# sz3/libcimbar

Hardware: AMD Instinct MI355X
Metric: decoded cimbar frames/s (1024x1024 mode-B) (higher is better)
Workload: dtype u8; 1 GPU; BASELINE configs[1]: 1024 clean mode-B frames per GPU per step, device-resident, bit-exact; distinct_input_batches=4, exchange_ranks=1, parallelism=frame-sharded x1; 3 steps in flight (pipelined entry point)

## Files before the change

### libcimbar_amd/csrc/host.hip.inc

```
struct CombineStream {
	DevBuf<uint8_t> symbols, colors, chunks; DevBuf<uint32_t> plane, flood, masks; DevBuf<int8_t> drift;
	DevBuf<uint32_t> weights;
	DevBuf<int> words;
	DevBuf<int> gsizes;
	Event ev_last;
	bool used = false;
	int min_agree = 0, max_group = 0;
	int vote = 0;
	CarryStore store() const { return CarryStore{symbols, colors, plane, drift, flood, chunks, masks, words, weights}; }
};

struct StitchStream {
	DevBuf<uint8_t> symbols, colors;
	DevBuf<uint32_t> usable;
	Event ev_last;
	bool used = false;
	bool carried = false;
	int cur = 0;
	StitchCarry carry() const { return StitchCarry{symbols, colors, usable, cur}; }
};

struct OnceStream {
	DevBuf<uint8_t> sig, row;
	DevBuf<uint32_t> words;
// ... 48 lines not shown
	DevBuf<uint8_t> d_rp_rchunks; DevBuf<uint32_t> d_rp_rmasks;
	int wave_adapt = 1;
	bool wave_ran = false;
	int wave_skip_left = 0;
	bool no_split_once = false;
	std::string err;
	Tables tb{};
	DevBuf<ushort2> tb_cell_xy; DevBuf<uint16_t> tb_stream_cell, tb_cell_grid, tb_ccm_grid; DevBuf<int16_t> tb_grid_cell, tb_cand;
	DevBuf<uint8_t> tb_stitch_line;
	DevBuf<uint16_t> tb_stitch_width;
	uint64_t tile_hashes[16] = {};
	int last_n = 0;
	int scan_n = 0;
	unsigned scan_w = 0, scan_h = 0;
	DevBuf<uint8_t> d_rgb;
	static constexpr int MAXP = 4;
	struct ScratchSet {
		int cap = 0;
		DevBuf<uint32_t> d_plane, d_cellmean;
		DevBuf<uint8_t> d_symbols, d_colors;
		DevBuf<int8_t> d_drift;
		DevBuf<uint32_t> d_flood;
		DevBuf<uint8_t> d_rs_ok;
		DevBuf<FrameState> d_states;
		DevBuf<float> d_ccm_frames, d_ccm_used;
		DevBuf<uint32_t> d_cmargin;
		int cm_cap = 0;
	} sets[MAXP];
	int pipe_depth = 3;
#ifdef CIMBAR_PROBES
	int dbg_skip = 0;
#else
	static constexpr int dbg_skip = 0;
#endif
	int pipe_set = 0;
	ScratchSet& cur() { return sets[pipe_set]; }
	bool pipe_used[MAXP] = {};
	Stream pstream_own[MAXP];
	hipStream_t pstream[MAXP] = {};
	Event ev_pk1[MAXP], ev_pdone[MAXP];
	Event ev_pgather[MAXP];
	bool pipe_gathered[MAXP] = {};
	struct FrameSlot {
		DevBuf<uint8_t> d_rgb;
		DevBuf<uint8_t> d_out;
		PinnedBuf<uint8_t> h_out;
		PinnedBuf<uint8_t> h_in;
		Event done;
		uint8_t* user_chunks = nullptr; uint32_t* user_mask = nullptr;
		long long ticket = -1;
	} fslot[MAXP];
	long long frame_tickets = 0;
	int k1_tall = -1;
	int k1_lds_pad = 0;
	size_t warp_scratch = (size_t)4 << 30;
	int warp_twopass = 1;
	DevBuf<int4> d_ex_box;
	DevBuf<uint8_t> d_ex_rgb;
	int frame_stage = 0;
	int frame_zerocopy = 1;
	int frame_copystream = 0;
	Stream fcopy;
	Event ev_fcopy[MAXP];
	struct FrameResult { long long ticket = -1; int rc = 0; } fresult[16];
	DevBuf<float> d_carry;
	DevBuf<uint8_t> d_template;
	DevBuf<uint8_t> d_gen_log;
	DevBuf<uint8_t> d_payload;
	DevBuf<uint8_t> d_chunks;
	DevBuf<uint32_t> d_masks;
	DevBuf<uint8_t> d_ex_in;
	const uint8_t* pad_src = nullptr; int pad_w = 0, pad_h = 0, pad_off = 0;
	DevBuf<uint8_t> d_ex_out;
	DevBuf<uint32_t> d_ex_hist; DevBuf<int> d_ex_thr; DevBuf<double> d_ex_minv;
	DevBuf<uint8_t> d_ex_gray;
	DevBuf<uint8_t> d_ex_frames;
	DevBuf<uint32_t> d_scan_hits; DevBuf<int> d_scan_nhits; DevBuf<ScanResult> d_scan_res;
	DevBuf<ScanAnchor> d_scan_serial;
	DevBuf<int> d_scan_offs, d_scan_ovf; DevBuf<ScanConf> d_scan_conf; DevBuf<ScanStage> d_scan_stage;
	PinnedBuf<double> h_ex_minv;
	Event ev_ex_minv;
	DevBuf<uint8_t> d_ud_img;
	DevBuf<int> d_ud_ok; DevBuf<double> d_ud_k1; DevBuf<int> d_ud_status;
	DevBuf<double> d_ud_xt; PinnedBuf<double> h_ud_xt;
	Event ev_ud_xt;
	size_t ud_scratch = (size_t)256 << 20;
	FloodScratch flood{};
	DevBuf<uint32_t> flood_heap, flood_next; DevBuf<uint8_t> flood_prio;
	int flood_cap = 0;
	DevBuf<uint32_t> d_fw_queue;
	int flood_verify = 0;
	DevBuf<uint8_t> d_vsym; DevBuf<int8_t> d_vdrift; DevBuf<uint32_t> d_vflag; int vcap = 0;
	DevBuf<unsigned long long> d_vtotals;
	int flood_dense_grid = 2048;
	int flood_dense = -1;
	int flood_wave = 1;
	int rf_threshold = -1, rf_fallback = 0;
	int rf_grid = FR_GRID;
	bool rf_valid = false;
	DevBuf<unsigned long long> d_rf_stats;
	bool timing = false;
	static constexpr int NSTAGE = 8;
	Event ev[NSTAGE + 1];
	float stage_ms[NSTAGE] = {};

	~cimbar_hip_ctx()
// ... 262 lines not shown
	ctx->vcap = 0;
	HIPCHK(ctx->d_vsym.reserve((size_t)n * NCELLS));
	HIPCHK(ctx->d_vdrift.reserve((size_t)n * NCELLS * 2));
	HIPCHK(ctx->d_vflag.reserve((size_t)n * 2));
	HIPCHK(hipMemset(ctx->d_vflag, 0xFF, sizeof(uint32_t) * (size_t)n * 2));
	if (!ctx->d_vtotals) { HIPCHK(ctx->d_vtotals.reserve(2)); HIPCHK(hipMemset(ctx->d_vtotals, 0, 2 * sizeof(unsigned long long))); }
	ctx->vcap = n;
	return 0;
}

int stage_input(cimbar_hip_ctx* ctx, hipStream_t st, DevBuf<uint8_t>& buf, const uint8_t* src, size_t bytes, int mem, const uint8_t** d)
{
	*d = src;
	if (mem == CIMBAR_HIP_MEM_HOST) {
		HIPCHK(buf.reserve(bytes));
		HIPCHK(hipMemcpyAsync(buf, src, bytes, hipMemcpyHostToDevice, st));
		*d = buf;
	}
	return 0;
}

int stage_output(cimbar_hip_ctx* ctx, DevBuf<uint8_t>& buf, uint8_t* dst, size_t bytes, int mem, uint8_t** d)
{
	*d = dst;
	if (mem == CIMBAR_HIP_MEM_HOST) {
		HIPCHK(buf.reserve(bytes));
		*d = buf;
	}
	return 0;
}

int drain_pipeline_into(cimbar_hip_ctx* ctx, hipStream_t st)
{
	for (int k = 0; k < cimbar_hip_ctx::MAXP; ++k)
		if (ctx->pipe_used[k]) HIPCHK(hipStreamWaitEvent(st, ctx->ev_pdone[k], 0));
	return 0;
}

void rotate_scratch_sets(cimbar_hip_ctx* ctx) { ctx->pipe_set = (ctx->pipe_set + 1) % ctx->pipe_depth; }

int ensure_flood_areas(cimbar_hip_ctx* ctx, int count)
{
	if (count <= ctx->flood_cap) return 0;
	HIPCHK(hipDeviceSynchronize());
	ctx->flood_cap = 0;
	HIPCHK(ctx->flood_heap.reserve((size_t)count * HEAP_CAP));
	HIPCHK(ctx->flood_prio.reserve((size_t)count * PRIO_STRIDE));
	if (!ctx->flood_next) { HIPCHK(ctx->flood_next.reserve((size_t)2 * FLOOD_COUNTERS)); HIPCHK(hipMemset(ctx->flood_next, 0, sizeof(uint32_t) * 2 * FLOOD_COUNTERS)); }
	ctx->flood = FloodScratch{ctx->flood_heap, ctx->flood_next, ctx->flood_prio};
	ctx->flood_cap = count;
	return 0;
}

constexpr int K1_TALL_MIN = 256;
constexpr int ERASURE_MAX_DEFAULT = RS_PARITY - 8;
inline int erasure_max(const cimbar_hip_ctx* ctx) { return ctx->er_max < 0 ? ERASURE_MAX_DEFAULT : ctx->er_max; }
inline int colour_erasure_max(const cimbar_hip_ctx* ctx) { return ctx->ec_max < 0 ? ERASURE_MAX_DEFAULT : ctx->ec_max; }

int enqueue(cimbar_hip_ctx* ctx, hipStream_t st, const uint8_t* d_rgb, int n, int pre, int cc, uint8_t* d_chunks, uint32_t* d_masks, int plain = 0,
            bool pipe = false, const int* d_sel = nullptr, int sel_stride = 0, bool symbols_only = false)
{
	cimbar_hip_ctx::ScratchSet& cur = ctx->cur();
	ctx->grp_valid = false;
	ctx->stitch_n = 0;
	ctx->gcv_valid = false;
	ctx->gcv_stream_n = -1;
	const bool colour_retry = !LEGACY && !plain && !symbols_only && ctx->ec_margin > 0;
	if (colour_retry) { if (int r = ensure_margin_capacity(ctx, cur)) return r; }
	ctx->cm_valid = colour_retry;
	const bool tm = ctx->timing && !pipe;
	int evi = 0;
	auto mark = [&]() -> hipError_t { return tm ? hipEventRecord(ctx->ev[evi++], st) : hipSuccess; };
	const dim3 cell_grid((NCELLS + 255) / 256, n);
	const int f0 = 0;

	uint32_t flagged[3] = {0, 0, 0};
	if (ctx->h_flagged) for (int k = 0; k < 3; ++k) flagged[k] = ((volatile uint32_t*)ctx->h_flagged)[k];
	const bool mostly_flood = flagged[1] != 0 && 4u * flagged[0] > flagged[1];
	const bool split = !tm && !pipe && ctx->tail_split && !ctx->no_split_once && !mostly_flood && n >= 64 * ctx->tail_parts;
	{
		const int areas_ = pipe ? FLOOD_GRID / ctx->pipe_depth : (split ? FLOOD_GRID / 2 : FLOOD_GRID);
		const int off_ = pipe ? (ctx->pipe_depth - 1) * areas_ : (split ? FLOOD_GRID / 2 : 0);
		int top = off_ + (n < areas_ ? n : areas_);
		if (ctx->flood_dense > 0 || (ctx->flood_dense < 0 && n > areas_)) top = FLOOD_DENSE_PER * off_ + (n < FLOOD_DENSE_PER * areas_ ? n : FLOOD_DENSE_PER * areas_);
		if (int r = ensure_flood_areas(ctx, top)) return r;
		if (ctx->flood_verify) if (int r = ensure_verify_capacity(ctx, n)) return r;
	}
	HIPCHK(mark());
	{
		dim3 g(K1_BLOCKS, n), gt(K1_TALL_BLOCKS, n);
		const bool pre_tall = ctx->k1_tall > 0 || (ctx->k1_tall < 0 && n >= K1_TALL_MIN);
		if (ctx->pad_src && n == 1) {
			uint8_t* frame = const_cast<uint8_t*>(d_rgb);
			const dim3 gp((IMG_W + 63) / 64, (IMG_H + 3) / 4);
			if (pre) hipLaunchKernelGGL((k_threshold_padded<3, true>), gp, dim3(256), 0, st, ctx->pad_src, ctx->pad_w, ctx->pad_h, ctx->pad_off, cur.d_plane, frame, cur.d_flood);
			else hipLaunchKernelGGL((k_threshold_padded<2, false>), gp, dim3(256), 0, st, ctx->pad_src, ctx->pad_w, ctx->pad_h, ctx->pad_off, cur.d_plane, frame, cur.d_flood);
			hipLaunchKernelGGL(k_cellmean_padded, dim3((GRID_CELLS + 255) / 256), dim3(256), 0, st, frame, cur.d_cellmean);
		} else if (d_sel) {
			if (pre_tall) hipLaunchKernelGGL((k_threshold<3, true, K1_TALLROWS>), gt, dim3(256), 0, st, d_rgb, cur.d_plane, cur.d_cellmean, cur.d_flood, f0, d_sel, sel_stride);
			else hipLaunchKernelGGL((k_threshold<3, true>), g, dim3(256), 0, st, d_rgb, cur.d_plane, cur.d_cellmean, cur.d_flood, f0, d_sel, sel_stride);
			hipLaunchKernelGGL((k_threshold<2, false>), g, dim3(256), 0, st, d_rgb, cur.d_plane, cur.d_cellmean, cur.d_flood, f0, d_sel, sel_stride);
		} else if (pre) {
			if (pre_tall) hipLaunchKernelGGL((k_threshold<3, true, K1_TALLROWS>), gt, dim3(256), 0, st, d_rgb, cur.d_plane, cur.d_cellmean, cur.d_flood, f0, (const int*)nullptr, 0);
			else hipLaunchKernelGGL((k_threshold<3, true>), g, dim3(256), 0, st, d_rgb, cur.d_plane, cur.d_cellmean, cur.d_flood, f0, (const int*)nullptr, 0);
		} else if (ctx->k1_tall > 0 || (ctx->k1_tall < 0 && pipe && n >= K1_TALL_MIN))
			hipLaunchKernelGGL((k_threshold<2, false, K1_TALLROWS>), dim3(K1_TALL_BLOCKS, n), dim3(256), (size_t)ctx->k1_lds_pad, st, d_rgb, cur.d_plane, cur.d_cellmean, cur.d_flood, f0, (const int*)nullptr, 0);
		else hipLaunchKernelGGL((k_threshold<2, false>), g, dim3(256), (size_t)ctx->k1_lds_pad, st, d_rgb, cur.d_plane, cur.d_cellmean, cur.d_flood, f0, (const int*)nullptr, 0);
	}
	HIPCHK(mark());
	const bool counted = !pipe && !tm && ctx->h_flagged && ctx->tail_split && n >= 64 * ctx->tail_parts;
	bool run_wave = ctx->flood_wave != 0;
	if (run_wave && counted && ctx->wave_adapt && !ctx->flood_verify) {
		if (ctx->wave_skip_left > 0) { --ctx->wave_skip_left; run_wave = false; }
		else if (ctx->wave_ran && flagged[0] >= 16u && 16u * (flagged[0] - (flagged[2] <= flagged[0] ? flagged[2] : flagged[0])) < flagged[0]) {
			run_wave = false;
			ctx->wave_skip_left = 14;
		}
	}
	if (counted) ctx->wave_ran = run_wave;
	const bool relaxed = !LEGACY && ctx->rf_threshold >= 0 && ctx->d_rf_stats && !(ctx->dbg_skip & 2);
	ctx->rf_valid = relaxed;
	auto tail = [&](hipStream_t s, int fa, int m, int part) -> hipError_t {
		if (part == 0) {
			if (!(ctx->dbg_skip & 1)) hipLaunchKernelGGL(k_symbols, dim3(K2_BLOCKS, m), dim3(256), 0, s, cur.d_plane, ctx->tb, cur.d_symbols, cur.d_flood, fa);
			if (hipError_t e = (s == st ? mark() : hipSuccess)) return e;
			const int areas = pipe ? FLOOD_GRID / ctx->pipe_depth : (split ? FLOOD_GRID / 2 : FLOOD_GRID);
			const int area0 = pipe ? ctx->pipe_set * areas : ((split && s != st) ? FLOOD_GRID / 2 : 0);
			if (run_wave && !(ctx->dbg_skip & 2)) {
				const int wareas = pipe ? FW_GRID / ctx->pipe_depth : (split ? FW_GRID / 2 : FW_GRID);
				const int warea0 = pipe ? ctx->pipe_set * wareas : ((split && s != st) ? FW_GRID / 2 : 0);
				hipLaunchKernelGGL(k_flood_wave, dim3(m < wareas ? m : wareas), dim3(256), 0, s, cur.d_plane, ctx->tb, ctx->d_fw_queue, cur.d_flood,
				                   cur.d_symbols, cur.d_drift, fa, m, warea0, cur.d_flood + cur.cap);
			} else if (ctx->flood_wave && !(ctx->dbg_skip & 2)) {
				if (hipError_t e = hipMemsetAsync(cur.d_flood + cur.cap + fa, 0xFF, sizeof(uint32_t) * (size_t)m, s)) return e;
			}
			const int counter = pipe ? ctx->pipe_set : ((split && s != st) ? 1 : 0);
			auto exact_flood = [&](const uint32_t* flags) {
				const int areas3 = areas * FLOOD_GRID3 / FLOOD_GRID;
				auto hand_out = [&](int grid) { if (grid < m) (void)hipMemsetAsync(ctx->flood.next + 2 * counter, 0, 2 * sizeof(uint32_t), s); return dim3(grid); };
				if (ctx->dbg_skip & 2) {}
				else if (ctx->flood_dense > 0 || (ctx->flood_dense < 0 && m > areas)) {
					const int areas8 = FLOOD_DENSE_PER * areas * ctx->flood_dense_grid / (FLOOD_DENSE_PER * FLOOD_GRID);
					hipLaunchKernelGGL((k_flood3<HEAP_LDS8, true>), hand_out(m < areas8 ? m : areas8), dim3(128), 0, s, cur.d_plane, ctx->tb, ctx->flood, flags, cur.d_symbols, cur.d_drift, fa, m,
					                   FLOOD_DENSE_PER * area0, counter);
				} else if (m <= areas3)
					hipLaunchKernelGGL((k_flood3<HEAP_LDS, false>), dim3(m), dim3(128), 0, s, cur.d_plane, ctx->tb, ctx->flood, flags, cur.d_symbols, cur.d_drift, fa, m, area0, counter);
				else
					hipLaunchKernelGGL((k_flood3<HEAP_LDS4, false>), hand_out(m < areas ? m : areas), dim3(128), 0, s, cur.d_plane, ctx->tb, ctx->flood, flags, cur.d_symbols, cur.d_drift, fa, m, area0, counter);
			};
			if (relaxed) {
				if (hipError_t e = hipMemsetAsync(cur.d_flood + 2 * cur.cap + fa, 0, sizeof(uint32_t) * (size_t)m, s)) return e;
				hipLaunchKernelGGL(k_flood_rounds, dim3(m < ctx->rf_grid ? m : ctx->rf_grid), dim3(FR_THREADS), 0, s, cur.d_plane, ctx->tb, cur.d_flood, cur.d_symbols,
				                   cur.d_drift, fa, m, (uint32_t)ctx->rf_threshold, cur.d_flood + 2 * cur.cap);
			} else exact_flood(cur.d_flood);
			if (ctx->flood_verify && ctx->flood_wave && !(ctx->dbg_skip & 2)) {
				hipLaunchKernelGGL(k_verify_begin, dim3(m), dim3(256), 0, s, cur.d_flood, cur.d_symbols, cur.d_drift, ctx->d_vflag, ctx->d_vsym, ctx->d_vdrift, fa, ctx->vcap);
				exact_flood(ctx->d_vflag);
				hipLaunchKernelGGL(k_verify_end, dim3(m), dim3(256), 0, s, cur.d_symbols, cur.d_drift, ctx->d_vflag, ctx->d_vsym, ctx->d_vdrift, fa, ctx->vcap, ctx->d_vtotals);
			}
			if (hipError_t e = (s == st ? mark() : hipSuccess)) return e;
// ... 103 lines not shown
{
	const int set = ctx->pipe_set;
	if (!ctx->pipe_used[set]) return false;
	*stream = ctx->pstream[set];
	*gathered = ctx->ev_pgather[set];
	ctx->pipe_gathered[set] = true;
	return true;
}

int cimbar_hip_create(int device, int mode_val, cimbar_hip_ctx** out)
{
	if (!out) return CIMBAR_HIP_EINVAL;
	*out = nullptr;
	if (mode_val != MODE_VAL) return CIMBAR_HIP_EINVAL;
	int count = 0;
	if (hipGetDeviceCount(&count) != hipSuccess || count <= 0 || device < 0 || device >= count) return CIMBAR_HIP_ENODEVICE;
	if (hipSetDevice(device) != hipSuccess) return CIMBAR_HIP_ENODEVICE;
	hipDeviceProp_t prop;
	if (hipGetDeviceProperties(&prop, device) != hipSuccess) return CIMBAR_HIP_ENODEVICE;
	if (std::strncmp(prop.gcnArchName, "gfx950", 6) != 0) return CIMBAR_HIP_ENODEVICE;

	cimbar_hip_ctx* ctx = new cimbar_hip_ctx();
	ctx->device = device;
	auto fail = [&](int code) { delete ctx; return code; };
	if (ctx->stream.create() != hipSuccess || ctx->stream2.create() != hipSuccess) return fail(CIMBAR_HIP_EHIP);
	if (const char* v = std::getenv("CIMBAR_HIP_PIPE_DEPTH")) { int k = std::atoi(v); if (k >= 2 && k <= cimbar_hip_ctx::MAXP) ctx->pipe_depth = k; }
	ctx->pstream[0] = ctx->stream;
	ctx->pstream[1] = ctx->stream2;
	for (int k = 2; k < ctx->pipe_depth; ++k) {
		if (ctx->pstream_own[k].create() != hipSuccess) return fail(CIMBAR_HIP_EHIP);
		ctx->pstream[k] = ctx->pstream_own[k];
	}
	for (Event* e : {&ctx->ev_k1, &ctx->ev_join})
		if (e->create() != hipSuccess) return fail(CIMBAR_HIP_EHIP);
	for (Event& e : ctx->ev_mid) if (e.create() != hipSuccess) return fail(CIMBAR_HIP_EHIP);
	for (Event& e : ctx->ev_pk1) if (e.create() != hipSuccess) return fail(CIMBAR_HIP_EHIP);
	for (Event& e : ctx->ev_pdone) if (e.create() != hipSuccess) return fail(CIMBAR_HIP_EHIP);
	for (Event& e : ctx->ev_pgather) if (e.create() != hipSuccess) return fail(CIMBAR_HIP_EHIP);
	if (const char* v = std::getenv("CIMBAR_HIP_TAIL_SPLIT")) ctx->tail_split = std::atoi(v);
	if (const char* v = std::getenv("CIMBAR_HIP_FLOOD_WAVE")) ctx->flood_wave = std::atoi(v) != 0;
	if (const char* v = std::getenv("CIMBAR_HIP_FLOOD_WAVE_ADAPT")) ctx->wave_adapt = std::atoi(v) != 0;
	if (const char* v = std::getenv("CIMBAR_HIP_FLOOD_VERIFY")) ctx->flood_verify = std::atoi(v) != 0;
	if (const char* v = std::getenv("CIMBAR_HIP_FLOOD_DENSE")) ctx->flood_dense = std::atoi(v);
	if (const char* v = std::getenv("CIMBAR_HIP_FLOOD_DENSE_GRID")) { int k = std::atoi(v); if (k >= 4 && k <= FLOOD_DENSE_PER * FLOOD_GRID) ctx->flood_dense_grid = k; }
	if (const char* v = std::getenv("CIMBAR_HIP_ROUNDS_GRID")) { int k = std::atoi(v); if (k >= 1 && k <= FR_GRID) ctx->rf_grid = k; }
#ifdef CIMBAR_PROBES
	if (const char* v = std::getenv("CIMBAR_HIP_DEBUG_SKIP")) ctx->dbg_skip = std::atoi(v);
#endif
	if (const char* v = std::getenv("CIMBAR_HIP_FRAME_STAGE")) ctx->frame_stage = std::atoi(v);
	if (const char* v = std::getenv("CIMBAR_HIP_WARP_TWOPASS")) ctx->warp_twopass = std::atoi(v);
	if (const char* v = std::getenv("CIMBAR_HIP_WARP_SCRATCH_MB")) { long k = std::atol(v); if (k >= 1 && k <= (1 << 20)) ctx->warp_scratch = (size_t)k << 20; }
	if (const char* v = std::getenv("CIMBAR_HIP_UNDISTORT_SCRATCH_MB")) { long k = std::atol(v); if (k >= 1 && k <= (1 << 20)) ctx->ud_scratch = (size_t)k << 20; }
	if (const char* v = std::getenv("CIMBAR_HIP_K1_STRIPS")) ctx->k1_tall = !std::strcmp(v, "tall") ? 1 : (!std::strcmp(v, "short") ? 0 : -1);
	if (const char* v = std::getenv("CIMBAR_HIP_K1_LDS_PAD")) { int k = std::atoi(v); if (k >= 0 && k <= 100000) ctx->k1_lds_pad = k; }
	if (const char* v = std::getenv("CIMBAR_HIP_FRAME_ZEROCOPY")) ctx->frame_zerocopy = std::atoi(v);
	if (const char* v = std::getenv("CIMBAR_HIP_FRAME_COPYSTREAM")) ctx->frame_copystream = std::atoi(v);
	if (const char* v = std::getenv("CIMBAR_HIP_TAIL_PARTS")) { int k = std::atoi(v); if (k >= 2 && k <= 8 && k % 2 == 0) ctx->tail_parts = k; }
	for (Event& e : ctx->ev) if (e.create(hipEventDefault) != hipSuccess) return fail(CIMBAR_HIP_EHIP);
	if (ctx->d_carry.reserve(10) != hipSuccess) return fail(CIMBAR_HIP_ENOMEM);
	if (hipMemset(ctx->d_carry, 0, sizeof(float) * 10) != hipSuccess) return fail(CIMBAR_HIP_EHIP);
	if (build_tables(ctx) != 0) return fail(CIMBAR_HIP_EHIP);
	if (ctx->h_flagged.reserve(4) == hipSuccess) { ctx->h_flagged[0] = ctx->h_flagged[1] = ctx->h_flagged[2] = 0; }
	else (void)hipGetLastError();
	*out = ctx;
	return CIMBAR_HIP_OK;
}

void cimbar_hip_destroy(cimbar_hip_ctx* ctx) { delete ctx; }

const char* cimbar_hip_last_error(const cimbar_hip_ctx* ctx) { return ctx ? ctx->err.c_str() : "null context"; }

int cimbar_hip_device(const cimbar_hip_ctx* ctx) { return ctx ? ctx->device : CIMBAR_HIP_EINVAL; }

int cimbar_hip_reset_ccm(cimbar_hip_ctx* ctx)
{
	if (!ctx) return CIMBAR_HIP_EINVAL;
	HIPCHK(hipSetDevice(ctx->device));
	HIPCHK(hipDeviceSynchronize());
	HIPCHK(hipMemsetAsync(ctx->d_carry, 0, sizeof(float) * 10, ctx->stream));
	HIPCHK(hipStreamSynchronize(ctx->stream));
	return 0;
}

int cimbar_hip_get_ccm(cimbar_hip_ctx* ctx, float out9[9])
{
	if (!ctx || !out9) return CIMBAR_HIP_EINVAL;
	float tmp[10];
	HIPCHK(hipSetDevice(ctx->device));
	HIPCHK(hipDeviceSynchronize());
	HIPCHK(hipMemcpy(tmp, ctx->d_carry, sizeof tmp, hipMemcpyDeviceToHost));
	std::memcpy(out9, tmp, sizeof(float) * 9);
	return tmp[9] != 0.0f ? 1 : 0;
}

int cimbar_hip_set_ccm(cimbar_hip_ctx* ctx, const float m9[9])
{
	if (!ctx || !m9) return CIMBAR_HIP_EINVAL;
	float tmp[10];
	std::memcpy(tmp, m9, sizeof(float) * 9);
	tmp[9] = 1.0f;
	HIPCHK(hipSetDevice(ctx->device));
	HIPCHK(hipDeviceSynchronize());
	HIPCHK(hipMemcpy(ctx->d_carry, tmp, sizeof tmp, hipMemcpyHostToDevice));
	return 0;
}

// ... 2012 lines not shown
```

### libcimbar_amd/csrc/k1_threshold.hip.inc

```
constexpr int k1_strips(int rows) { return (DIM_Y + rows - 1) / rows; }
constexpr int k1_blocks(int rows) { return (k1_strips(rows) + 3) / 4; }
constexpr int K1_STRIPS = k1_strips(K1_CELLROWS);
constexpr int K1_BLOCKS = k1_blocks(K1_CELLROWS), K1_TALL_BLOCKS = k1_blocks(K1_TALLROWS);
constexpr int GRID_CELLS = DIM_X * DIM_Y;

constexpr int K1_NP = K1_PPL / 2, K1_NDW = K1_PPL * 3 / 4;
constexpr bool K1_PARTIAL = LAST_PX != K1_PPL;
static_assert(K1_PPL == 16 || K1_PPL == 12, "16 pixels (3 x dwordx4) or 12 pixels (3 x dwordx3) per lane");
static_assert(!K1_PARTIAL || (K1_PPL == 12 && LAST_PX == 4), "a partial last lane holds exactly its first load (four pixels)");

struct RowOff { uint32_t o0, o1, o2; };
__device__ __forceinline__ RowOff row_offsets(int lane)
{
	if (LAST_LANE != 63) lane = lane < LAST_LANE ? lane : LAST_LANE;
	RowOff r;
	r.o0 = (uint32_t)lane * (K1_PPL * 3);
	const bool whole = !K1_PARTIAL || lane < LAST_LANE;
	r.o1 = whole ? r.o0 + K1_PPL : r.o0;
	r.o2 = whole ? r.o0 + 2 * K1_PPL : r.o0;
	return r;
}
template <int PPL> struct RowSrc;
template <> struct RowSrc<16> {
	const uint8_t* frame;
	__device__ __forceinline__ explicit RowSrc(const uint8_t* f) : frame(f) {}
};
template <> struct RowSrc<12> {
	__amdgpu_buffer_rsrc_t rsrc;
	__device__ __forceinline__ explicit RowSrc(const uint8_t* f) : rsrc(__builtin_amdgcn_make_buffer_rsrc(const_cast<uint8_t*>(f), 0, (int)FRAME_RGB, 0x00020000)) {}
};
__device__ __forceinline__ void load_row(const RowSrc<16>& src, int r, const RowOff& ro, uint32_t (&d)[12])
{
	const uint4* p = reinterpret_cast<const uint4*>(src.frame + (size_t)r * (IMG_W * 3) + ro.o0);
	uint4 a = p[0], b = p[1], c = p[2];
	d[0] = a.x; d[1] = a.y; d[2] = a.z; d[3] = a.w;
	d[4] = b.x; d[5] = b.y; d[6] = b.z; d[7] = b.w;
	d[8] = c.x; d[9] = c.y; d[10] = c.z; d[11] = c.w;
}
__device__ __forceinline__ void load_row(const RowSrc<12>& src, int r, const RowOff& ro, uint32_t (&d)[9])
{
	typedef uint32_t u3 __attribute__((ext_vector_type(3)));
	const int so = __builtin_amdgcn_readfirstlane(r * (IMG_W * 3));
	const u3 a = __builtin_amdgcn_raw_buffer_load_b96(src.rsrc, (int)ro.o0, so, 0);
	const u3 b = __builtin_amdgcn_raw_buffer_load_b96(src.rsrc, (int)ro.o1, so, 0);
	const u3 c = __builtin_amdgcn_raw_buffer_load_b96(src.rsrc, (int)ro.o2, so, 0);
	d[0] = a.x; d[1] = a.y; d[2] = a.z;
	d[3] = b.x; d[4] = b.y; d[5] = b.z;
	d[6] = c.x; d[7] = c.y; d[8] = c.z;
}

template <int PPL, bool BGR = false>
__device__ __forceinline__ void gray_T(const uint32_t* d, uint32_t* T)
{
	constexpr uint32_t LO2 = BGR ? 46u | (70u << 8) | (140u << 16) : 140u | (70u << 8) | (46u << 16);
	constexpr uint32_t HI = BGR ? 29u | (150u << 8) | (76u << 16) : 76u | (150u << 8) | (29u << 16);
	constexpr int NDW = PPL * 3 / 4;
#pragma unroll
	for (int p = 0; p < PPL; ++p) {
		const int w = (3 * p) >> 2, sh = (3 * p) & 3;
		uint32_t v;
		const bool IN_PLACE = sh == 1;
		if (sh == 0 || IN_PLACE) v = d[w];
		else if (w == NDW - 1) v = d[NDW - 1] >> (8 * sh);
		else v = __builtin_amdgcn_alignbyte(d[w + 1], d[w], sh);
		const uint32_t lo = __builtin_amdgcn_udot4(v, IN_PLACE ? LO2 << 8 : LO2, 32768u, false);
		const uint32_t hi = __builtin_amdgcn_udot4(v, IN_PLACE ? HI << 8 : HI, 0u, false);
		T[p] = (hi << 8) + lo;
	}
}
__device__ __forceinline__ void gray16_T(const uint32_t d[12], uint32_t T[16]) { gray_T<16>(d, T); }
template <int NP>
__device__ __forceinline__ void pairs_T(const uint32_t* T, uint32_t* G)
{
#pragma unroll
	for (int i = 0; i < NP; ++i) G[i] = __builtin_amdgcn_perm(T[i + NP], T[i], 0x0c060c02u);
}
__device__ __forceinline__ void pairs_from_T(const uint32_t T[16], uint32_t G[8]) { pairs_T<8>(T, G); }

__device__ __forceinline__ uint32_t from_left_lane(uint32_t v, uint32_t edge) { return (uint32_t)__builtin_amdgcn_update_dpp((int)edge, (int)v, 0x138, 0xf, 0xf, false); }
__device__ __forceinline__ uint32_t from_right_lane(uint32_t v, uint32_t edge) { return (uint32_t)__builtin_amdgcn_update_dpp((int)edge, (int)v, 0x130, 0xf, 0xf, false); }
__device__ __forceinline__ uint32_t from_right_lane_row(uint32_t v, uint32_t edge)
{
	const uint32_t r = from_right_lane(v, edge);
	if (LAST_LANE == 63) return r;
	return (int)(threadIdx.x & 63) == LAST_LANE ? edge : r;
}


struct EdgeSel { uint32_t keep_lo, all, reflect; };
__device__ __forceinline__ EdgeSel edge_selectors(int lane)
{
	EdgeSel e;
	const bool last = K1_PARTIAL && lane >= LAST_LANE;
	e.keep_lo = last ? 0x05040100u : 0x03020100u;
	e.all = last ? 0x05040504u : 0x03020100u;
	e.reflect = last ? 0x03020504u : 0x03020100u;
	return e;
}
template <bool P = K1_PARTIAL, int LP = LAST_PX>
__device__ __forceinline__ void patch_reflect(uint32_t (&G)[K1_NP], const EdgeSel& e)
{
	if constexpr (P) {
// ... 21 lines not shown
	for (int i = 0; i < NP; ++i) {
		const uint32_t w = i == 0 ? W0 : gc[i - 1], e = i == NP - 1 ? E7 : gc[i + 1];
		const uint32_t sum = gn[i] + gs[i] + w + e;
		const uint32_t t = gc[i] * 9u + 0x10001000u - 2u * sum;
		uint32_t q = (t >> 1) & 0x7FFF7FFFu;
		q += t & q & 0x00010001u;
		us2 v = __builtin_bit_cast(us2, q);
		const us2 lo = {2048, 2048}, hi = {2048 + 255, 2048 + 255};
		v = __builtin_elementwise_min(__builtin_elementwise_max(v, lo), hi);
		G[i] = __builtin_bit_cast(uint32_t, v) - 0x08000800u;
	}
}

template <int RAD, int SLOT>
__device__ __forceinline__ uint32_t box_row(uint32_t (&ring)[2 * RAD + 2][K1_NP], uint32_t (&C)[K1_NP], const uint32_t (&G)[K1_NP], bool emit)
{
	constexpr int RING = 2 * RAD + 2, R = 2 * RAD + 1, N = R * R, NP = K1_NP;
	constexpr int OLD = (SLOT + 1) % RING;
	constexpr int CTR = (SLOT + RING - RAD) % RING;
#pragma unroll
	for (int i = 0; i < NP; ++i) {
		C[i] += G[i] - ring[OLD][i];
		ring[SLOT][i] = G[i];
	}
	if (!emit) return 0;

	uint32_t X[NP + 2 * RAD];
#pragma unroll
	for (int i = 0; i < NP; ++i) X[RAD + i] = C[i];
#pragma unroll
	for (int k = 1; k <= RAD; ++k) {
		const uint32_t left = from_left_lane(C[NP - k] >> 16, C[0] & 0xFFFFu);
		X[RAD - k] = left | (C[NP - k] << 16);
		const uint32_t right = from_right_lane_row(C[k - 1] & 0xFFFFu, C[NP - 1] >> 16);
		X[RAD + NP - 1 + k] = (C[k - 1] >> 16) | (right << 16);
	}
	constexpr uint32_t K = (0x8000u - (uint32_t)(N / 2) - 1u) * 0x00010001u;
	uint32_t KS = K;
#pragma unroll
	for (int k = 0; k < R; ++k) KS -= X[k];
	uint32_t M = 0;
#pragma unroll
	for (int i = 0; i < NP; ++i) {
		if (i > 0) KS += X[i - 1] - X[i + 2 * RAD];
		const uint32_t r = __umul24(ring[CTR][i], (uint32_t)N) + KS;
		M |= (r >> i) & (0x80008000u >> i);
	}
	if constexpr (NP == 8) return (M & 0xFF00u) | (M >> 24);
	else return ((M >> (16 - 2 * NP)) & (((1u << NP) - 1u) << NP)) | (M >> (32 - NP));
}

__device__ __forceinline__ void row_order_fence() { asm volatile("" ::: "memory"); }

template <int RAD, bool PRE, int ROWS = K1_CELLROWS>
#ifndef K1_WAVES
#define K1_WAVES 3
#endif
#ifndef K1_PRE_WAVES
#define K1_PRE_WAVES 2
#endif
#ifndef K1_PRE_DEPTH
#define K1_PRE_DEPTH 4
#endif
__global__ __launch_bounds__(256, PRE ? K1_PRE_WAVES : K1_WAVES) void k_threshold(const uint8_t* __restrict__ rgb, uint32_t* __restrict__ plane,
                                                                uint32_t* __restrict__ cellmean, uint32_t* __restrict__ flood_flag, int f0,
                                                                const int* __restrict__ sel, int sel_stride)
{
	constexpr int RING = 2 * RAD + 2;
	if (sel != nullptr && (sel[(size_t)(f0 + blockIdx.y) * sel_stride] == 2) != PRE) return;
	__shared__ __attribute__((aligned(16))) uint16_t s_col[4][64 * K1_PPL * 3];
	constexpr int NP = K1_NP, NDW = K1_NDW;
	const int lane = threadIdx.x & 63;
	const int wave = __builtin_amdgcn_readfirstlane(threadIdx.x >> 6);
	const int strip = blockIdx.x * 4 + wave;
	constexpr int STRIPS = k1_strips(ROWS);
	if (strip >= STRIPS) return;
	const int f = f0 + blockIdx.y;
	const uint8_t* frame = rgb + (size_t)f * FRAME_RGB;
	uint32_t* out = plane + (size_t)f * PLANE_WORDS;
	uint32_t* cm = cellmean + (size_t)f * GRID_CELLS;
	const int y_begin = strip == 0 ? 0 : OFFSET + strip * ROWS * PITCH;
	const int y_end = strip == STRIPS - 1 ? IMG_H : OFFSET + (strip + 1) * ROWS * PITCH;
	const int total = (y_end - y_begin) + 2 * RAD;
	if (strip == 0 && lane == 0) flood_flag[f] = 0;

	const RowOff ro = row_offsets(lane);
	const RowSrc<K1_PPL> src(frame);
	const EdgeSel es = edge_selectors(lane);
	uint32_t ring[RING][NP];
	uint32_t C[NP];
	uint32_t acc_e[NDW], acc_o[NDW];
#pragma unroll
	for (int k = 0; k < RING; ++k)
#pragma unroll
		for (int i = 0; i < NP; ++i) ring[k][i] = 0;
#pragma unroll
	for (int i = 0; i < NP; ++i) C[i] = 0;
#pragma unroll
	for (int k = 0; k < NDW; ++k) { acc_e[k] = 0; acc_o[k] = 0; }

	auto clampy = [](int y) { return y < 0 ? 0 : (y >= IMG_H ? IMG_H - 1 : y); };
	const int dir = (strip & 1) ? -1 : 1;
	const int y_first = dir > 0 ? y_begin - RAD : y_end - 1 + RAD;
	const int y_stop = dir > 0 ? y_end - 1 + RAD : y_begin - RAD;
#ifndef K1_DEPTH
#define K1_DEPTH 3
#endif
	constexpr int DEPTH = PRE ? K1_PRE_DEPTH : K1_DEPTH;
	static_assert(RING % DEPTH == 0, "prefetch depth must divide the ring size");
	uint32_t buf[DEPTH][NDW];
	auto bounded = [&](int y) { return clampy(dir > 0 ? (y < y_stop ? y : y_stop) : (y > y_stop ? y : y_stop)); };
	auto ahead = [&](int t) {
		const int a = bounded(y_first + dir * t) + dir;
		return a < 0 ? 1 : (a >= IMG_H ? IMG_H - 2 : a);
	};
	uint32_t GR[4][NP];
	if (PRE) {
		static_assert(!PRE || RING % 4 == 0, "gray ring period must divide the box ring");
		const int y0 = clampy(y_first), yb = y0 - dir;
		uint32_t d0[NDW], d1[NDW], T[K1_PPL];
		load_row(src, yb < 0 ? 1 : (yb >= IMG_H ? IMG_H - 2 : yb), ro, d0);
		load_row(src, y0, ro, d1);
#pragma unroll
		for (int k = 0; k < DEPTH; ++k) { load_row(src, ahead(k), ro, buf[k]); row_order_fence(); }
		gray_T<K1_PPL>(d0, T); pairs_T<NP>(T, GR[3]); patch_reflect(GR[3], es);
		gray_T<K1_PPL>(d1, T); pairs_T<NP>(T, GR[0]); patch_reflect(GR[0], es);
#pragma unroll
		for (int i = 0; i < NP; ++i) { GR[1][i] = 0; GR[2][i] = 0; }
	} else {
#pragma unroll
		for (int k = 0; k < DEPTH; ++k) { load_row(src, clampy(y_first + dir * k), ro, buf[k]); row_order_fence(); }
	}

	auto step = [&](const int s, const int t) __attribute__((always_inline)) {
		const int y = y_first + dir * t;
		uint32_t (&d)[NDW] = buf[s % DEPTH];
		uint32_t G[NP];
		int yl = y;
		if (PRE) {
			yl = ahead(t);
			uint32_t T[K1_PPL];
			gray_T<K1_PPL>(d, T);
			pairs_T<NP>(T, GR[(s + 1) & 3]);
			patch_reflect(GR[(s + 1) & 3], es);
			sharp_pairs(GR[(s + 3) & 3], GR[s & 3], GR[(s + 1) & 3], G);
			if (bounded(y + dir) == bounded(y)) {
#pragma unroll
				for (int i = 0; i < NP; ++i) { GR[(s + 1) & 3][i] = GR[s & 3][i]; GR[s & 3][i] = GR[(s + 3) & 3][i]; }
			}
		} else {
			uint32_t T[K1_PPL];
			gray_T<K1_PPL>(d, T);
			pairs_T<NP>(T, G);
		}
		patch_edge(G, es);

		const bool in_grid = yl >= y_begin && yl < y_end && yl >= OFFSET + 1 && yl < OFFSET + DIM_Y * PITCH;
		const int ph = in_grid ? (yl - OFFSET) % PITCH : 0;
#ifdef K1_PROBE_NOCOLOR
		if (false) {
#else
		if (ph >= 1 && ph <= 6) {
#endif
#pragma unroll
			for (int k = 0; k < NDW; ++k) {
				acc_e[k] += d[k] & 0x00FF00FFu;
				acc_o[k] += __builtin_amdgcn_perm(0u, d[k], 0x0c030c01u);
			}
		}
		load_row(src, PRE ? ahead(t + DEPTH) : bounded(y + dir * DEPTH), ro, d);

#ifdef K1_PROBE_NOCOLOR
		if (false) {
#else
		if (ph == (dir > 0 ? 6 : 1)) {
#endif
			uint16_t* sc = s_col[wave];
			uint32_t w[2 * NDW];
#pragma unroll
			for (int k = 0; k < NDW; ++k) {
				w[2 * k] = (acc_e[k] & 0xFFFFu) | (acc_o[k] << 16);
				w[2 * k + 1] = (acc_e[k] >> 16) | (acc_o[k] & 0xFFFF0000u);
				acc_e[k] = 0; acc_o[k] = 0;
			}
			if constexpr (K1_PPL == 16) {
				typedef uint32_t u4 __attribute__((ext_vector_type(4)));
				const uint32_t at = (uint32_t)(uintptr_t)(sc + 48 * lane);
#pragma unroll
				for (int j = 0; j < NDW / 2; ++j) {
					const u4 v = {w[4 * j], w[4 * j + 1], w[4 * j + 2], w[4 * j + 3]};
					asm volatile("ds_write_b128 %0, %1 offset:%2" :: "v"(at), "v"(v), "n"(16 * j) : "memory");
				}
			} else {
				typedef uint32_t u2 __attribute__((ext_vector_type(2)));
				const uint32_t at = (uint32_t)(uintptr_t)(sc + K1_PPL * 3 * lane);
#pragma unroll
				for (int k = 0; k < NDW; ++k) {
					const u2 v = {w[2 * k], w[2 * k + 1]};
					asm volatile("ds_write_b64 %0, %1 offset:%2" :: "v"(at), "v"(v), "n"(8 * k) : "memory");
				}
			}
			__builtin_amdgcn_fence(__ATOMIC_RELEASE, "wavefront");
			__builtin_amdgcn_wave_barrier();
			const int cell_row = (yl - OFFSET) / PITCH;
#pragma unroll
			for (int half = 0; half < 2; ++half) {
				const int c = lane + 64 * half;
				if (c < DIM_X) {
					const uint16_t* src = sc + 3 * (PITCH * c + OFFSET + 1);
					uint32_t r = 0, gg = 0, b = 0;
#pragma unroll
					for (int k = 0; k < 6; ++k) { r += src[3 * k]; gg += src[3 * k + 1]; b += src[3 * k + 2]; }
					cm[cell_row * DIM_X + c] = (r / 36u) | ((gg / 36u) << 8) | ((b / 36u) << 16);
				}
			}
			__builtin_amdgcn_wave_barrier();
		}

		uint32_t bits = 0;
		const bool emit = t >= 2 * RAD;
		switch (s) {
			case 0: bits = box_row<RAD, 0>(ring, C, G, emit); break;
			case 1: bits = box_row<RAD, 1>(ring, C, G, emit); break;
			case 2: bits = box_row<RAD, 2>(ring, C, G, emit); break;
			case 3: bits = box_row<RAD, 3>(ring, C, G, emit); break;
			case 4: bits = box_row<RAD, 4>(ring, C, G, emit); break;
			case 5: bits = box_row<RAD, 5>(ring, C, G, emit); break;
			case 6: bits = box_row<RAD, 6 % RING>(ring, C, G, emit); break;
			default: bits = box_row<RAD, 7 % RING>(ring, C, G, emit); break;
		}
		if (emit) {
			uint32_t* orow = out + (size_t)(y - dir * RAD) * PLANE_ROW;
			if constexpr (K1_PPL == 16) {
				const uint32_t nb = (uint32_t)__builtin_amdgcn_update_dpp(0, (int)bits, 0xB1, 0xf, 0xf, true);
				const uint32_t w0 = (lane & 1) ? ((nb << 16) | bits) : ((bits << 16) | nb);
				const uint32_t w1 = (uint32_t)__builtin_amdgcn_update_dpp(0, (int)w0, 0x4E, 0xf, 0xf, true);
				const uint32_t w2 = (uint32_t)__builtin_amdgcn_update_dpp(0, (int)w0, 0x104, 0xf, 0xf, true);
				const uint32_t w3 = (uint32_t)__builtin_amdgcn_update_dpp(0, (int)w1, 0x104, 0xf, 0xf, true);
				if (!(lane & 7)) {
					uint4 v; v.x = w0; v.y = w1; v.z = w2; v.w = w3;
					*reinterpret_cast<uint4*>(orow + (lane >> 3) * 4) = v;
				}
			} else {
				const uint32_t nb = (uint32_t)__builtin_amdgcn_update_dpp(0, (int)bits, 0xB1, 0xf, 0xf, true);
				const uint32_t c24 = (bits << 12) | nb;
				const uint32_t o24 = (uint32_t)__builtin_amdgcn_update_dpp(0, (int)c24, 0x4E, 0xf, 0xf, true);
				const uint32_t hi16 = c24 >> 8, lo32 = (c24 << 24) | o24;
				const uint32_t bh = (uint32_t)__builtin_amdgcn_update_dpp(0, (int)hi16, 0x104, 0xf, 0xf, true);
				const uint32_t bl = (uint32_t)__builtin_amdgcn_update_dpp(0, (int)lo32, 0x104, 0xf, 0xf, true);
				if (!(lane & 7)) {
					struct __attribute__((packed, aligned(4))) W3 { uint32_t x, y, z; } v;
					v.x = (hi16 << 16) | (lo32 >> 16); v.y = (lo32 << 16) | bh; v.z = bl;
					*reinterpret_cast<W3*>(orow + (lane >> 3) * 3) = v;
				}
			}
		}
	};
	static_assert(PITCH + 2 * RAD >= RING, "a strip's shortest walk covers a full pass over the ring");
	int t0 = 0;
	do {
#pragma unroll
		for (int s = 0; s < RING; ++s) step(s, t0 + s);
		t0 += RING;
	} while (t0 + RING <= total);
#pragma unroll
	for (int s = 0; s < RING - 1; ++s) {
		if (t0 + s >= total) return;
		step(s, t0 + s);
	}
}
```

Baseline: 1.354 million frames/s.

## Stream threshold-kernel input rows through LDS with direct global-to-LDS loads

Adds a k_threshold_lds variant in which each wave prefetches its source rows straight into shared memory using global_load_lds_dwordx4, optionally with non-temporal hints, then reads them back with ds_read_b128 instead of keeping a register prefetch ring. To make room in LDS, the colour transpose now runs in two halves over 32 lanes. In mode 68 the tall-strip plain path uses the non-temporal LDS variant by default, and an environment variable selects it elsewhere. The aim is to cut VGPR pressure and use wider loads, at the cost of more LDS use (which may lower occupancy), extra waitcnt serialisation and an extra LDS round trip.

```diff
diff --git a/libcimbar_amd/csrc/host.hip.inc b/libcimbar_amd/csrc/host.hip.inc
--- a/libcimbar_amd/csrc/host.hip.inc
+++ b/libcimbar_amd/csrc/host.hip.inc
@@ -124,6 +124,7 @@
 	} fslot[MAXP];
 	long long frame_tickets = 0;
 	int k1_tall = -1;
+	int k1_loads = -1;
 	int k1_lds_pad = 0;
 	size_t warp_scratch = (size_t)4 << 30;
 	int warp_twopass = 1;
@@ -492,6 +493,19 @@
 	return 0;
 }
 
+template <int ROWS>
+void launch_k1_plain(const cimbar_hip_ctx* ctx, hipStream_t st, int n, const uint8_t* d_rgb, uint32_t* plane, uint32_t* cellmean, uint32_t* flood, int f0, const int* d_sel, int sel_stride)
+{
+	const dim3 g(k1_blocks(ROWS), n);
+	const size_t pad = d_sel ? 0 : (size_t)ctx->k1_lds_pad;
+	if constexpr (K1_PPL == 16) {
+		const int loads = ctx->k1_loads >= 0 ? ctx->k1_loads : (ROWS == K1_TALLROWS && ROWS != K1_CELLROWS ? K1_LOADS_TALL : K1_LOADS_SHORT);
+		if (loads == 1) { hipLaunchKernelGGL((k_threshold_lds<ROWS, false>), g, dim3(256), pad, st, d_rgb, plane, cellmean, flood, f0, d_sel, sel_stride); return; }
+		if (loads == 2) { hipLaunchKernelGGL((k_threshold_lds<ROWS, true>), g, dim3(256), pad, st, d_rgb, plane, cellmean, flood, f0, d_sel, sel_stride); return; }
+	}
+	hipLaunchKernelGGL((k_threshold<2, false, ROWS>), g, dim3(256), pad, st, d_rgb, plane, cellmean, flood, f0, d_sel, sel_stride);
+}
+
 constexpr int K1_TALL_MIN = 256;
 constexpr int ERASURE_MAX_DEFAULT = RS_PARITY - 8;
 inline int erasure_max(const cimbar_hip_ctx* ctx) { return ctx->er_max < 0 ? ERASURE_MAX_DEFAULT : ctx->er_max; }
@@ -539,13 +553,13 @@
 		} else if (d_sel) {
 			if (pre_tall) hipLaunchKernelGGL((k_threshold<3, true, K1_TALLROWS>), gt, dim3(256), 0, st, d_rgb, cur.d_plane, cur.d_cellmean, cur.d_flood, f0, d_sel, sel_stride);
 			else hipLaunchKernelGGL((k_threshold<3, true>), g, dim3(256), 0, st, d_rgb, cur.d_plane, cur.d_cellmean, cur.d_flood, f0, d_sel, sel_stride);
-			hipLaunchKernelGGL((k_threshold<2, false>), g, dim3(256), 0, st, d_rgb, cur.d_plane, cur.d_cellmean, cur.d_flood, f0, d_sel, sel_stride);
+			launch_k1_plain<K1_CELLROWS>(ctx, st, n, d_rgb, cur.d_plane, cur.d_cellmean, cur.d_flood, f0, d_sel, sel_stride);
 		} else if (pre) {
 			if (pre_tall) hipLaunchKernelGGL((k_threshold<3, true, K1_TALLROWS>), gt, dim3(256), 0, st, d_rgb, cur.d_plane, cur.d_cellmean, cur.d_flood, f0, (const int*)nullptr, 0);
 			else hipLaunchKernelGGL((k_threshold<3, true>), g, dim3(256), 0, st, d_rgb, cur.d_plane, cur.d_cellmean, cur.d_flood, f0, (const int*)nullptr, 0);
 		} else if (ctx->k1_tall > 0 || (ctx->k1_tall < 0 && pipe && n >= K1_TALL_MIN))
-			hipLaunchKernelGGL((k_threshold<2, false, K1_TALLROWS>), dim3(K1_TALL_BLOCKS, n), dim3(256), (size_t)ctx->k1_lds_pad, st, d_rgb, cur.d_plane, cur.d_cellmean, cur.d_flood, f0, (const int*)nullptr, 0);
-		else hipLaunchKernelGGL((k_threshold<2, false>), g, dim3(256), (size_t)ctx->k1_lds_pad, st, d_rgb, cur.d_plane, cur.d_cellmean, cur.d_flood, f0, (const int*)nullptr, 0);
+			launch_k1_plain<K1_TALLROWS>(ctx, st, n, d_rgb, cur.d_plane, cur.d_cellmean, cur.d_flood, f0, nullptr, 0);
+		else launch_k1_plain<K1_CELLROWS>(ctx, st, n, d_rgb, cur.d_plane, cur.d_cellmean, cur.d_flood, f0, nullptr, 0);
 	}
 	HIPCHK(mark());
 	const bool counted = !pipe && !tm && ctx->h_flagged && ctx->tail_split && n >= 64 * ctx->tail_parts;
@@ -755,6 +769,7 @@
 	if (const char* v = std::getenv("CIMBAR_HIP_WARP_SCRATCH_MB")) { long k = std::atol(v); if (k >= 1 && k <= (1 << 20)) ctx->warp_scratch = (size_t)k << 20; }
 	if (const char* v = std::getenv("CIMBAR_HIP_UNDISTORT_SCRATCH_MB")) { long k = std::atol(v); if (k >= 1 && k <= (1 << 20)) ctx->ud_scratch = (size_t)k << 20; }
 	if (const char* v = std::getenv("CIMBAR_HIP_K1_STRIPS")) ctx->k1_tall = !std::strcmp(v, "tall") ? 1 : (!std::strcmp(v, "short") ? 0 : -1);
+	if (const char* v = std::getenv("CIMBAR_HIP_K1_LOADS")) ctx->k1_loads = !std::strcmp(v, "lds") ? 1 : (!std::strcmp(v, "lds-nt") ? 2 : (!std::strcmp(v, "regs") ? 0 : -1));
 	if (const char* v = std::getenv("CIMBAR_HIP_K1_LDS_PAD")) { int k = std::atoi(v); if (k >= 0 && k <= 100000) ctx->k1_lds_pad = k; }
 	if (const char* v = std::getenv("CIMBAR_HIP_FRAME_ZEROCOPY")) ctx->frame_zerocopy = std::atoi(v);
 	if (const char* v = std::getenv("CIMBAR_HIP_FRAME_COPYSTREAM")) ctx->frame_copystream = std::atoi(v);
diff --git a/libcimbar_amd/csrc/k1_threshold.hip.inc b/libcimbar_amd/csrc/k1_threshold.hip.inc
--- a/libcimbar_amd/csrc/k1_threshold.hip.inc
+++ b/libcimbar_amd/csrc/k1_threshold.hip.inc
@@ -48,6 +48,42 @@
 	d[3] = b.x; d[4] = b.y; d[5] = b.z;
 	d[6] = c.x; d[7] = c.y; d[8] = c.z;
 }
+constexpr int K1_ROWBYTES = IMG_W * 3;
+constexpr int K1_LOADS_TALL = MODE_VAL == 68 ? 2 : 0, K1_LOADS_SHORT = 0;
+template <bool NT> struct RowSrcLds {
+	const uint8_t* frame;
+	uint32_t voff, slots, rd;
+	__device__ __forceinline__ RowSrcLds(const uint8_t* f, int lane, uint32_t wave_slots) : voff(16u * lane), slots(wave_slots), rd(wave_slots + 48u * lane)
+	{
+		const uint64_t a = (uint64_t)(uintptr_t)f;
+		frame = reinterpret_cast<const uint8_t*>((uint64_t)(uint32_t)__builtin_amdgcn_readfirstlane((int)(a >> 32)) << 32 | (uint32_t)__builtin_amdgcn_readfirstlane((int)a));
+	}
+	template <int SLOT> __device__ __forceinline__ void issue(int r) const
+	{
+		const uint8_t* row = frame + (uint32_t)__builtin_amdgcn_readfirstlane(r * K1_ROWBYTES);
+		uint32_t keep;
+#define K1_LDS_ROW(POLICY) \
+		asm volatile("s_mov_b32 %0, m0\n\ts_mov_b32 m0, %3\n\ts_nop 2\n\t" \
+		             "global_load_lds_dwordx4 %1, %2" POLICY "\n\t" \
+		             "global_load_lds_dwordx4 %1, %2 offset:1024" POLICY "\n\t" \
+		             "global_load_lds_dwordx4 %1, %2 offset:2048" POLICY "\n\t" \
+		             "s_mov_b32 m0, %0" : "=&s"(keep) : "v"(voff), "s"(row), "s"(slots + (uint32_t)(SLOT * K1_ROWBYTES)) : "memory")
+		if constexpr (NT) K1_LDS_ROW(" nt"); else K1_LDS_ROW("");
+#undef K1_LDS_ROW
+	}
+	template <int SLOT, int N> __device__ __forceinline__ void read(uint32_t (&d)[12]) const
+	{
+		typedef uint32_t u4 __attribute__((ext_vector_type(4)));
+		u4 a, b, c;
+		asm volatile("s_waitcnt vmcnt(%4)\n\t"
+		             "ds_read_b128 %0, %3 offset:%5\n\tds_read_b128 %1, %3 offset:%6\n\tds_read_b128 %2, %3 offset:%7\n\t"
+		             "s_waitcnt lgkmcnt(0)"
+		             : "=&v"(a), "=&v"(b), "=&v"(c) : "v"(rd), "i"(N), "i"(SLOT * K1_ROWBYTES), "i"(SLOT * K1_ROWBYTES + 16), "i"(SLOT * K1_ROWBYTES + 32) : "memory");
+		d[0] = a.x; d[1] = a.y; d[2] = a.z; d[3] = a.w;
+		d[4] = b.x; d[5] = b.y; d[6] = b.z; d[7] = b.w;
+		d[8] = c.x; d[9] = c.y; d[10] = c.z; d[11] = c.w;
+	}
+};
 
 template <int PPL, bool BGR = false>
 __device__ __forceinline__ void gray_T(const uint32_t* d, uint32_t* T)
@@ -175,7 +211,6 @@
 
 __device__ __forceinline__ void row_order_fence() { asm volatile("" ::: "memory"); }
 
-template <int RAD, bool PRE, int ROWS = K1_CELLROWS>
 #ifndef K1_WAVES
 #define K1_WAVES 3
 #endif
@@ -185,13 +220,22 @@
 #ifndef K1_PRE_DEPTH
 #define K1_PRE_DEPTH 4
 #endif
-__global__ __launch_bounds__(256, PRE ? K1_PRE_WAVES : K1_WAVES) void k_threshold(const uint8_t* __restrict__ rgb, uint32_t* __restrict__ plane,
-                                                                uint32_t* __restrict__ cellmean, uint32_t* __restrict__ flood_flag, int f0,
-                                                                const int* __restrict__ sel, int sel_stride)
+#ifndef K1_DEPTH
+#define K1_DEPTH 3
+#endif
+template <int RAD, bool PRE, int ROWS, int LOADS>
+__device__ __forceinline__ void k1_threshold_body(const uint8_t* __restrict__ rgb, uint32_t* __restrict__ plane, uint32_t* __restrict__ cellmean,
+                                                  uint32_t* __restrict__ flood_flag, int f0, const int* __restrict__ sel, int sel_stride)
 {
 	constexpr int RING = 2 * RAD + 2;
 	if (sel != nullptr && (sel[(size_t)(f0 + blockIdx.y) * sel_stride] == 2) != PRE) return;
-	__shared__ __attribute__((aligned(16))) uint16_t s_col[4][64 * K1_PPL * 3];
+	constexpr bool LDSROWS = LOADS != 0;
+	static_assert(!LDSROWS || (!PRE && K1_PPL == 16 && IMG_W == 1024), "rows through LDS: the plain instances of the 1024-pixel modes");
+	constexpr int DEPTH = PRE ? K1_PRE_DEPTH : K1_DEPTH;
+	static_assert(RING % DEPTH == 0, "prefetch depth must divide the ring size");
+	constexpr int COL_LANES = LDSROWS ? 32 : 64;
+	__shared__ __attribute__((aligned(16))) uint16_t s_col[4][COL_LANES * K1_PPL * 3];
+	__shared__ __attribute__((aligned(16))) uint8_t s_rows[LDSROWS ? 4 * DEPTH * K1_ROWBYTES : 16];
 	constexpr int NP = K1_NP, NDW = K1_NDW;
 	const int lane = threadIdx.x & 63;
 	const int wave = __builtin_amdgcn_readfirstlane(threadIdx.x >> 6);
@@ -226,12 +270,19 @@
 	const int dir = (strip & 1) ? -1 : 1;
 	const int y_first = dir > 0 ? y_begin - RAD : y_end - 1 + RAD;
 	const int y_stop = dir > 0 ? y_end - 1 + RAD : y_begin - RAD;
-#ifndef K1_DEPTH
-#define K1_DEPTH 3
-#endif
-	constexpr int DEPTH = PRE ? K1_PRE_DEPTH : K1_DEPTH;
-	static_assert(RING % DEPTH == 0, "prefetch depth must divide the ring size");
-	uint32_t buf[DEPTH][NDW];
+	uint32_t buf[LDSROWS ? 1 : DEPTH][NDW];
+	const uint32_t wave_slots = LDSROWS ? (uint32_t)__builtin_amdgcn_readfirstlane((int)(uint32_t)(uintptr_t)(s_rows + wave * (DEPTH * K1_ROWBYTES))) : 0u;
+	const RowSrcLds<LOADS == 2> lsrc(frame, lane, wave_slots);
+	auto lds_issue = [&](const int k, const int r) __attribute__((always_inline)) {
+		switch (k) {
+			case 0: lsrc.template issue<0>(r); break;
+			case 1: lsrc.template issue<1 % DEPTH>(r); break;
+			case 2: lsrc.template issue<2 % DEPTH>(r); break;
+			case 3: lsrc.template issue<3 % DEPTH>(r); break;
+			case 4: lsrc.template issue<4 % DEPTH>(r); break;
+			default: lsrc.template issue<5 % DEPTH>(r); break;
+		}
+	};
 	auto bounded = [&](int y) { return clampy(dir > 0 ? (y < y_stop ? y : y_stop) : (y > y_stop ? y : y_stop)); };
 	auto ahead = [&](int t) {
 		const int a = bounded(y_first + dir * t) + dir;
@@ -250,6 +301,9 @@
 		gray_T<K1_PPL>(d1, T); pairs_T<NP>(T, GR[0]); patch_reflect(GR[0], es);
 #pragma unroll
 		for (int i = 0; i < NP; ++i) { GR[1][i] = 0; GR[2][i] = 0; }
+	} else if constexpr (LDSROWS) {
+#pragma unroll
+		for (int k = 0; k < DEPTH; ++k) lds_issue(k, clampy(y_first + dir * k));
 	} else {
 #pragma unroll
 		for (int k = 0; k < DEPTH; ++k) { load_row(src, clampy(y_first + dir * k), ro, buf[k]); row_order_fence(); }
@@ -257,7 +311,24 @@
 
 	auto step = [&](const int s, const int t) __attribute__((always_inline)) {
 		const int y = y_first + dir * t;
-		uint32_t (&d)[NDW] = buf[s % DEPTH];
+		uint32_t dl[NDW];
+		uint32_t (&d)[NDW] = LDSROWS ? dl : buf[s % (LDSROWS ? 1 : DEPTH)];
+		if constexpr (LDSROWS) {
+			constexpr int N_LOADS = 3 * (DEPTH - 1);
+			auto rd = [&](auto slot) __attribute__((always_inline)) {
+				if (t >= 2 * RAD + DEPTH) lsrc.template read<decltype(slot)::value, N_LOADS + DEPTH>(dl);
+				else lsrc.template read<decltype(slot)::value, N_LOADS>(dl);
+			};
+			switch (s % DEPTH) {
+				case 0: rd(std::integral_constant<int, 0>()); break;
+				case 1: rd(std::integral_constant<int, 1 % DEPTH>()); break;
+				case 2: rd(std::integral_constant<int, 2 % DEPTH>()); break;
+				case 3: rd(std::integral_constant<int, 3 % DEPTH>()); break;
+				case 4: rd(std::integral_constant<int, 4 % DEPTH>()); break;
+				default: rd(std::integral_constant<int, 5 % DEPTH>()); break;
+			}
+			lds_issue(s % DEPTH, bounded(y + dir * DEPTH));
+		}
 		uint32_t G[NP];
 		int yl = y;
 		if (PRE) {
@@ -291,7 +362,7 @@
 				acc_o[k] += __builtin_amdgcn_perm(0u, d[k], 0x0c030c01u);
 			}
 		}
-		load_row(src, PRE ? ahead(t + DEPTH) : bounded(y + dir * DEPTH), ro, d);
+		if constexpr (!LDSROWS) load_row(src, PRE ? ahead(t + DEPTH) : bounded(y + dir * DEPTH), ro, buf[s % (LDSROWS ? 1 : DEPTH)]);
 
 #ifdef K1_PROBE_NOCOLOR
 		if (false) {
@@ -306,6 +377,33 @@
 				w[2 * k + 1] = (acc_e[k] >> 16) | (acc_o[k] & 0xFFFF0000u);
 				acc_e[k] = 0; acc_o[k] = 0;
 			}
+			if constexpr (LDSROWS) {
+				static_assert(DIM_X == 112 && OFFSET + PITCH * 55 + 6 < 512 && OFFSET + PITCH * 56 + 1 >= 512, "the halves of the colour transpose hold disjoint cells");
+				typedef uint32_t u4 __attribute__((ext_vector_type(4)));
+				const uint32_t at = (uint32_t)(uintptr_t)(sc + 48 * (lane & 31));
+				const int cell_row = (yl - OFFSET) / PITCH;
+#pragma unroll
+				for (int half = 0; half < 2; ++half) {
+					if ((lane >> 5) == half) {
+#pragma unroll
+						for (int j = 0; j < NDW / 2; ++j) {
+							const u4 v = {w[4 * j], w[4 * j + 1], w[4 * j + 2], w[4 * j + 3]};
+							asm volatile("ds_write_b128 %0, %1 offset:%2" :: "v"(at), "v"(v), "n"(16 * j) : "memory");
+						}
+					}
+					__builtin_amdgcn_fence(__ATOMIC_RELEASE, "wavefront");
+					__builtin_amdgcn_wave_barrier();
+					if (lane < DIM_X / 2) {
+						const int c = lane + (DIM_X / 2) * half;
+						const uint16_t* src = sc + 3 * (PITCH * c + OFFSET + 1 - 512 * half);
+						uint32_t r = 0, gg = 0, b = 0;
+#pragma unroll
+						for (int k = 0; k < 6; ++k) { r += src[3 * k]; gg += src[3 * k + 1]; b += src[3 * k + 2]; }
+						cm[cell_row * DIM_X + c] = (r / 36u) | ((gg / 36u) << 8) | ((b / 36u) << 16);
+					}
+					__builtin_amdgcn_wave_barrier();
+				}
+			} else {
 			if constexpr (K1_PPL == 16) {
 				typedef uint32_t u4 __attribute__((ext_vector_type(4)));
 				const uint32_t at = (uint32_t)(uintptr_t)(sc + 48 * lane);
@@ -338,6 +436,7 @@
 				}
 			}
 			__builtin_amdgcn_wave_barrier();
+			}
 		}
 
 		uint32_t bits = 0;
@@ -386,9 +485,25 @@
 		for (int s = 0; s < RING; ++s) step(s, t0 + s);
 		t0 += RING;
 	} while (t0 + RING <= total);
+	auto done = [&]() __attribute__((always_inline)) { if constexpr (LDSROWS) asm volatile("s_waitcnt vmcnt(0)" ::: "memory"); };
 #pragma unroll
 	for (int s = 0; s < RING - 1; ++s) {
-		if (t0 + s >= total) return;
+		if (t0 + s >= total) { done(); return; }
 		step(s, t0 + s);
 	}
-}
+	done();
+}
+
+template <int RAD, bool PRE, int ROWS = K1_CELLROWS>
+__global__ __launch_bounds__(256, PRE ? K1_PRE_WAVES : K1_WAVES) void k_threshold(const uint8_t* __restrict__ rgb, uint32_t* __restrict__ plane,
+                                                                uint32_t* __restrict__ cellmean, uint32_t* __restrict__ flood_flag, int f0,
+                                                                const int* __restrict__ sel, int sel_stride)
+{
+	k1_threshold_body<RAD, PRE, ROWS, 0>(rgb, plane, cellmean, flood_flag, f0, sel, sel_stride);
+}
+template <int ROWS, bool NT>
+__global__ __launch_bounds__(256, K1_WAVES) void k_threshold_lds(const uint8_t* __restrict__ rgb, uint32_t* __restrict__ plane, uint32_t* __restrict__ cellmean,
+                                                                 uint32_t* __restrict__ flood_flag, int f0, const int* __restrict__ sel, int sel_stride)
+{
+	k1_threshold_body<2, false, ROWS, NT ? 2 : 1>(rgb, plane, cellmean, flood_flag, f0, sel, sel_stride);
+}
```

After: 1.372 million frames/s (median of 6 runs). 1.01x the previous value.
